# Alabuta/RaytracingInOneWeekend

Measured on AMD Instinct MI355X. Metric: Mrays/sec + frame wall-clock, huge-scene 1280x720x128spp @1/2/4/8 GPU, higher is better.
Workload: dtype f32; 1 GPU; huge-scene 1280x720x128spp (BASELINE config 3); scene=huge (486 spheres), width=1280, height=720, spp=128, max_depth=64, camera=reference, kernel=exact (bit-exact), cull, parallelism=row-interleaved x1, RCCL gather of f32 tiles, output=f32, hw_queues=8, hw_queues_env=4, deep_split=8, deep_min_items=33554432

## Files before the change

### include/rt_api.h

```cpp
#ifndef RT_API_H
#define RT_API_H

#include <stddef.h>
#include <stdint.h>

#ifdef __cplusplus
extern "C" {
#endif

#define RT_API_VERSION 2

enum rt_status {
    RT_OK = 0,
    RT_ERR_INVALID = -1,
    RT_ERR_DEVICE = -2,
    RT_ERR_CAPACITY = -3,
    RT_ERR_UNSUPPORTED = -4,
    RT_ERR_COMM = -5,
    RT_ERR_IO = -6
};

typedef struct rt_sphere {
    float center[3];
    float radius;
// ... 58 lines not shown
    uint32_t transpose_max;
    uint32_t wave_queue_rays;
    uint32_t diag;
    uint64_t ring_pass_bytes;
} rt_options;
enum rt_diag {
    RT_DIAG_IEEE_ROOTS = 1u << 0,
    RT_DIAG_NO_SHORTCUT = 1u << 1,
    RT_DIAG_NO_NEIGHBOURS = 1u << 2,
    RT_DIAG_NO_ROOT_BOX = 1u << 3,
    RT_DIAG_SHADE_LDS = 1u << 4,
    RT_DIAG_SHADE_GLOBAL = 1u << 5,
    RT_DIAG_STATS = 1u << 6,
    RT_DIAG_STATS_DEEP_ONLY = 1u << 7,
    RT_DIAG_VERBOSE = 1u << 8,
    RT_DIAG_STANDIN_TRANSPORT = 1u << 9,
    RT_DIAG_UNBOUNDED_NB = 1u << 10,
    RT_DIAG_NO_PAIRS = 1u << 11,
    RT_DIAG_PAIRS = 1u << 12,
    RT_DIAG_IN_FLIGHT = 1u << 13,
    RT_DIAG_NATURAL_ORDER = 1u << 14,
    RT_DIAG_NO_SKY = 1u << 15,
    RT_DIAG_LONE_UNSPLIT = 1u << 16,
    RT_DIAG_SKY_SERIAL = 1u << 17
};
int rt_options_default(rt_options *out);
int rt_options_parse(const char *text, rt_options *inout);
int rt_set_default_options(const rt_options *options);
int rt_get_default_options(rt_options *out);

int rt_camera_init(const float position[3], const float lookat[3], const float up[3],
                   float aspect, float vfov_degrees, float aperture, float focus_distance,
                   uint32_t mode, rt_camera *out);
int rt_camera_default(uint32_t width, uint32_t height, uint32_t mode, rt_camera *out);
int rt_scene_simple(rt_sphere *spheres, uint32_t sphere_cap, uint32_t *n_spheres,
                    rt_material *materials, uint32_t material_cap, uint32_t *n_materials);
int rt_scene_cuda(rt_sphere *spheres, uint32_t sphere_cap, uint32_t *n_spheres,
                  rt_material *materials, uint32_t material_cap, uint32_t *n_materials);
int rt_camera_cuda(uint32_t width, uint32_t height, rt_camera *out);
int rt_scene_huge(uint32_t seed, rt_sphere *spheres, uint32_t sphere_cap, uint32_t *n_spheres,
                  rt_material *materials, uint32_t material_cap, uint32_t *n_materials);

int rt_tile_order(const rt_sphere *spheres, uint32_t n_spheres, const rt_material *materials,
                  uint32_t n_materials, const rt_camera *camera, const rt_params *params,
                  uint32_t *perm, uint32_t cap, uint32_t *n_blocks, uint32_t *n_lead, uint32_t *n_sky);

int rt_release_cached(void);
int rt_render_f32(const rt_sphere *spheres, uint32_t n_spheres,
                  const rt_material *materials, uint32_t n_materials,
                  const rt_camera *camera, const rt_params *params,
                  float *rgb_out, rt_stats *stats);
int rt_render_rgb8(const rt_sphere *spheres, uint32_t n_spheres,
                   const rt_material *materials, uint32_t n_materials,
                   const rt_camera *camera, const rt_params *params,
                   uint8_t *rgb_out, rt_stats *stats);
int rt_render_multi_f32(const rt_sphere *spheres, uint32_t n_spheres,
                        const rt_material *materials, uint32_t n_materials,
                        const rt_camera *camera, const rt_params *params, int ngpu,
                        float *rgb_out, rt_stats *stats);
int rt_render_multi_rgb8(const rt_sphere *spheres, uint32_t n_spheres,
                         const rt_material *materials, uint32_t n_materials,
                         const rt_camera *camera, const rt_params *params, int ngpu,
                         uint8_t *rgb_out, rt_stats *stats);

int rt_write_ppm(const char *path, const uint8_t *rgb, uint32_t width, uint32_t height);

int rt_render_cuda_impl(uint32_t width, uint32_t height, uint8_t *rgb_out);

// ... 99 lines not shown
```

### raytracinginoneweekend_amd/__init__.py

```python
from . import _abi as abi
from ._lib import RtError, lib
from .camera import CORRECTED, REFERENCE, Camera
from .render import (DeviceScene, MultiContext, default_options, default_options_set, denoise,
                     denoise_device, denoise_params,
                     epilogue_rgb8_device, make_params, options, parse_options, render_aov, render_cuda_impl, render_f32,
                     release_cached, render_multi_f32, render_multi_rgb8, render_rgb8, save_ppm,
                     set_default_options, tile_order)
from .scene import (Dielectric, Lambert, Metal, RaytracerData, Sphere, cuda_scene_arrays, huge_scene,
                    huge_scene_arrays, simple_scene, simple_scene_arrays)

__version__ = "0.1.0"
```

### raytracinginoneweekend_amd/_abi.py

```python
import ctypes as C

import numpy as np

RT_OK = 0
RT_ERR_INVALID = -1
RT_ERR_DEVICE = -2
RT_ERR_CAPACITY = -3
RT_ERR_UNSUPPORTED = -4
RT_ERR_COMM = -5
RT_ERR_IO = -6

RT_OUTPUT_F32, RT_OUTPUT_RGB8 = 0, 1

RT_LAMBERT, RT_METAL, RT_DIELECTRIC = 0, 1, 2
RT_CAMERA_REFERENCE, RT_CAMERA_CORRECTED = 0, 1

RT_FLAG_FULL_FRAME = 1 << 0
RT_FLAG_FAST_MATH = 1 << 1
RT_FLAG_SCALAR_SCENE = 1 << 2
RT_FLAG_BRUTE_FORCE = 1 << 3
RT_FLAG_CUDA_COMPAT = 1 << 4
RT_FLAG_WAVEFRONT = 1 << 5

RT_DENOISE_DEMODULATE = 1 << 0
# ... 32 lines not shown
class RtOptions(C.Structure):
    _fields_ = [
        ("size", C.c_uint32), ("render_streams", C.c_uint32), ("workspaces_per_stream", C.c_uint32),
        ("deep_split", C.c_uint32), ("max_pass_bytes", C.c_uint64), ("max_workspace_bytes", C.c_uint64),
        ("deep_min_items", C.c_uint64), ("cluster_size", C.c_uint32), ("transpose_max", C.c_uint32),
        ("wave_queue_rays", C.c_uint32), ("diag", C.c_uint32), ("ring_pass_bytes", C.c_uint64),
    ]


class RtSceneUsage(C.Structure):
    _fields_ = [
        ("device_bytes", C.c_uint64), ("workspace_bytes", C.c_uint64), ("render_streams", C.c_uint32),
        ("workspaces", C.c_uint32), ("pass_samples", C.c_uint32), ("static_lds_bytes", C.c_uint32),
        ("max_lds_bytes", C.c_uint32), ("deep_launch", C.c_uint32), ("pair_passes", C.c_uint32),
        ("split_passes", C.c_uint32), ("lead_tiles", C.c_uint32), ("sky_tiles", C.c_uint32),
    ]


RT_DIAG = {
    "ieee_roots": 1 << 0, "no_shortcut": 1 << 1, "no_neighbours": 1 << 2, "no_root_box": 1 << 3,
    "shade_lds": 1 << 4, "shade_global": 1 << 5, "stats": 1 << 6, "stats_deep_only": 1 << 7, "verbose": 1 << 8,
    "standin_transport": 1 << 9, "unbounded_nb": 1 << 10, "no_pairs": 1 << 11, "pairs": 1 << 12,
    "in_flight": 1 << 13, "natural_order": 1 << 14, "no_sky": 1 << 15, "lone_unsplit": 1 << 16,
    "sky_serial": 1 << 17,
}


class RtStats(C.Structure):
    _fields_ = [
        ("primaries", C.c_uint64), ("segments", C.c_uint64), ("sphere_tests", C.c_uint64),
        ("box_tests", C.c_uint64),
        ("kernel_ms", C.c_double), ("wall_ms", C.c_double),
    ]


class RtAovBuffers(C.Structure):
    _fields_ = [
        ("size", C.c_uint32), ("samples", C.c_uint32),
        ("albedo", C.c_void_p), ("normal", C.c_void_p), ("depth", C.c_void_p), ("alpha", C.c_void_p),
        ("sphere_id", C.c_void_p),
    ]


class RtDenoiseParams(C.Structure):
    _fields_ = [
        ("size", C.c_uint32), ("width", C.c_uint32), ("height", C.c_uint32), ("levels", C.c_uint32),
        ("sigma_color", C.c_float), ("sigma_normal", C.c_float), ("sigma_depth", C.c_float),
# ... 59 lines not shown
```

### raytracinginoneweekend_amd/_lib.py

```python
import ctypes as C
import os

from . import _abi as abi

PKG = os.path.dirname(os.path.abspath(__file__))
LIB_PATH = os.environ.get("RT_LIB_PATH") or os.path.join(PKG, "librt_mi355x.so")

_lib = None


class RtError(RuntimeError):

    def __init__(self, status, message):
        super().__init__(f"rt status {status}: {message}")
        self.status = status


def _declare(L):
    P = C.POINTER
    sig = {
        "rt_version": (C.c_int, []),
        "rt_last_error": (C.c_char_p, []),
        "rt_device_count": (C.c_int, [P(C.c_int)]),
        "rt_camera_init": (C.c_int, [P(C.c_float), P(C.c_float), P(C.c_float), C.c_float, C.c_float,
                                     C.c_float, C.c_float, C.c_uint32, P(abi.RtCamera)]),
        "rt_camera_default": (C.c_int, [C.c_uint32, C.c_uint32, C.c_uint32, P(abi.RtCamera)]),
        "rt_scene_simple": (C.c_int, [P(abi.RtSphere), C.c_uint32, P(C.c_uint32), P(abi.RtMaterial),
                                      C.c_uint32, P(C.c_uint32)]),
        "rt_scene_huge": (C.c_int, [C.c_uint32, P(abi.RtSphere), C.c_uint32, P(C.c_uint32),
                                    P(abi.RtMaterial), C.c_uint32, P(C.c_uint32)]),
        "rt_scene_cuda": (C.c_int, [P(abi.RtSphere), C.c_uint32, P(C.c_uint32), P(abi.RtMaterial),
                                    C.c_uint32, P(C.c_uint32)]),
        "rt_camera_cuda": (C.c_int, [C.c_uint32, C.c_uint32, P(abi.RtCamera)]),
        "rt_render_cuda_impl": (C.c_int, [C.c_uint32, C.c_uint32, P(C.c_uint8)]),
        "rt_release_cached": (C.c_int, []),
        "rt_tile_order": (C.c_int, [P(abi.RtSphere), C.c_uint32, P(abi.RtMaterial), C.c_uint32, P(abi.RtCamera),
                                    P(abi.RtParams), P(C.c_uint32), C.c_uint32, P(C.c_uint32), P(C.c_uint32),
                                    P(C.c_uint32)]),
        "rt_render_f32": (C.c_int, [P(abi.RtSphere), C.c_uint32, P(abi.RtMaterial), C.c_uint32,
                                    P(abi.RtCamera), P(abi.RtParams), P(C.c_float), P(abi.RtStats)]),
        "rt_render_rgb8": (C.c_int, [P(abi.RtSphere), C.c_uint32, P(abi.RtMaterial), C.c_uint32,
                                     P(abi.RtCamera), P(abi.RtParams), P(C.c_uint8), P(abi.RtStats)]),
        "rt_render_multi_f32": (C.c_int, [P(abi.RtSphere), C.c_uint32, P(abi.RtMaterial), C.c_uint32,
                                          P(abi.RtCamera), P(abi.RtParams), C.c_int, P(C.c_float),
                                          P(abi.RtStats)]),
        "rt_render_multi_rgb8": (C.c_int, [P(abi.RtSphere), C.c_uint32, P(abi.RtMaterial), C.c_uint32,
                                           P(abi.RtCamera), P(abi.RtParams), C.c_int, P(C.c_uint8),
                                           P(abi.RtStats)]),
        "rt_write_ppm": (C.c_int, [C.c_char_p, P(C.c_uint8), C.c_uint32, C.c_uint32]),
        "rt_multi_create": (C.c_int, [P(abi.RtSphere), C.c_uint32, P(abi.RtMaterial), C.c_uint32, P(C.c_int),
                                      C.c_int, P(C.c_void_p)]),
        "rt_multi_destroy": (C.c_int, [C.c_void_p]),
        "rt_multi_info": (C.c_int, [C.c_void_p, P(C.c_int), P(C.c_int)]),
        "rt_multi_render_device": (C.c_int, [C.c_void_p, P(abi.RtCamera), P(abi.RtParams), C.c_uint32, C.c_void_p,
                                             C.c_void_p]),
        "rt_multi_render_f32": (C.c_int, [C.c_void_p, P(abi.RtCamera), P(abi.RtParams), P(C.c_float),
                                          P(abi.RtStats)]),
        "rt_multi_render_rgb8": (C.c_int, [C.c_void_p, P(abi.RtCamera), P(abi.RtParams), P(C.c_uint8),
                                           P(abi.RtStats)]),
        "rt_scene_create": (C.c_int, [P(abi.RtSphere), C.c_uint32, P(abi.RtMaterial), C.c_uint32, C.c_int,
                                      P(C.c_void_p)]),
# ... 60 lines not shown
```

### raytracinginoneweekend_amd/csrc/rt_consts.h

```cpp
#pragma once
#include <stdint.h>

namespace rt {

struct UDiv {
    uint32_t m, s1, s2;
};

constexpr float kIsoR2Grow = 1.0201f;
constexpr uint32_t kShortcut = 0x80000000u;
#ifndef RT_SUPER
#define RT_SUPER 8
#endif
constexpr uint32_t kSuperClusters = RT_SUPER;
static_assert(kSuperClusters % 2 == 0, "clusters are tested in pairs");

}
```

### raytracinginoneweekend_amd/csrc/rt_device.h

```cpp
#pragma once
#include <hip/hip_runtime.h>
#include <stdint.h>

#include "rt_consts.h"

namespace rt {

struct FrameConsts {
    float org[3], llc[3], hor[3], ver[3];
    float lens, fW, fH;
    uint32_t corrected, W, spp;
    uint32_t inc_data_lo, inc_data_hi, inc_cam_lo, inc_cam_hi;
    uint32_t row_offset, row_stride, tiled_rows, tiles_x, n_pixels, sample_begin;
    UDiv div_W, div_tiles_x, div_n_pixels;
    uint32_t tile_lw;
    float rW, rH;
    uint32_t div_fast;
    uint32_t n_pairs;
};

constexpr uint32_t kItSlot = (1u << 29) - 1u;
constexpr uint32_t kItSecond = 1u << 31;
constexpr uint32_t kItFirstDeep = 1u << 30;
constexpr uint32_t kItRestart = 1u << 29;
// ... 25 lines not shown
    uint32_t full_frame;
    uint64_t inc_data, inc_cam;
    uint32_t n_pixels, tiles_x, tiled_rows;
    uint32_t tile_lw;
    uint32_t sample_begin, sample_end;
    uint32_t n_items;
    uint32_t n_slots;
    uint32_t n_pair_items;
    uint32_t n_blocks;
    float guided_l2b;
    uint32_t n_spheres, n_materials;
    const float4 *blob;
    uint32_t blob_units;
    uint32_t n_geo, n_always, n_clusters, clus_offset;
    uint32_t n_supers, supers_offset;
    uint32_t use_root;
    uint32_t iso;
    uint32_t transpose_max;
    uint32_t fast_roots;
    float clus_pad;
    uint32_t shade_offset;
    uint32_t lds_units;
    uint32_t shade_lds;
    float *slots;
    uint32_t *queue_ctr;
    unsigned long long *segments;
    unsigned long long *dbg;
    DeepQueue deep;
    uint32_t deep_depth;
    uint32_t deep_mode;
    uint32_t deep_prio;
    uint32_t deep_static;
    uint32_t diag_unbounded_nb;
    const uint32_t *block_perm;
    uint32_t n_groups;
    uint32_t grp_pix[4];
    uint32_t grp_items[3];
    uint32_t grp_blocks[3];
    UDiv div_grp[3];
};

constexpr uint32_t kDbgError = 15;
enum BoundsCode : uint32_t {
    BC_NONE = 0, BC_HINT_NB = 1, BC_SHADE = 2, BC_SLOT = 3, BC_DEEP_APPEND = 4, BC_DEEP_ITEM = 5,
    BC_DEEP_HINT = 6, BC_MEMBERS = 7, BC_DEEP_PX = 8
};
// ... 93 lines not shown
```

### raytracinginoneweekend_amd/csrc/rt_host.cpp

```cpp
#include <dlfcn.h>
#include <hip/hip_runtime.h>
#include <rccl/rccl.h>

#include <algorithm>
#include <cerrno>
#include <cfloat>
#include <chrono>
#include <cmath>
#include <cstdint>
#include <cstdio>
#include <cstdlib>
#include <cstring>
#include <map>
#include <mutex>
#include <random>
#include <string>
#include <vector>

#include "../../include/rt_api.h"
#include "rt_device.h"
#include "rt_host_build.h"

using namespace rthost;

// ... 64 lines not shown
#define RT_SHORT_OTHERS -1
#endif
int grid_wg_per_cu(int occ, bool in_flight, uint32_t streams, uint64_t pass_items)
{
    if (!in_flight) return occ;
    const int short_others = RT_SHORT_OTHERS > 0 ? RT_SHORT_OTHERS : std::max(1, static_cast<int>(streams) - 1);
    const int others = pass_items <= kShortPassItems ? short_others
                                                     : std::min(2, std::max(1, static_cast<int>(streams) - 1));
    return std::max(1, (occ + others - 1) / others);
}

}

struct rt_scene {
    int device = 0;
    rt_options opt{};
    uint32_t n_spheres = 0, n_materials = 0;
    float *blob[2] = {nullptr, nullptr};
    uint32_t blob_units[2] = {0, 0}, n_geo[2] = {0, 0}, n_always[2] = {0, 0}, n_clusters[2] = {0, 0},
             clus_offset[2] = {0, 0};
    float clus_pad[2] = {0.f, 0.f};
    uint32_t n_supers[2] = {0, 0}, supers_offset[2] = {0, 0};
    uint32_t shade_offset[2] = {0, 0};
    bool in_fast_range = false;
    float *slots[kMaxWs] = {};
    size_t slots_bytes[kMaxWs] = {};
    float *acc = nullptr;
    size_t acc_bytes = 0;
    void *deep[kMaxWs] = {};
    size_t deep_bytes[kMaxWs] = {}, deep_clean[kMaxWs] = {};
    size_t deep_meet_at[kMaxWs] = {};
    unsigned long long *deep_over = nullptr, *deep_over_dev = nullptr;
    static constexpr size_t kDeepOffKeys = 8;
    static constexpr uint64_t kDeepOffCalls = 256;
    std::vector<std::pair<unsigned long long, uint64_t>> deep_off;
    void *wq = nullptr;
    size_t wq_bytes = 0;
    int occ_wave[2] = {-1, -1};
    uint32_t *queue_ctr = nullptr;
    hipStream_t xs[kMaxBufs] = {};
    hipEvent_t ev_done[kMaxWs] = {}, ev_free[kMaxWs] = {};
    hipEvent_t ev_main[kMaxWs] = {};
    hipEvent_t ev_sky = nullptr;
    bool free_valid[kMaxWs] = {};
    bool ctr_dirty[kMaxWs];
    rt_scene() { std::fill(std::begin(ctr_dirty), std::end(ctr_dirty), true); }
// ... 195 lines not shown

extern "C" {


int rt_scene_destroy(rt_scene *sc)
{
    if (!sc) return RT_OK;
    int prev = 0;
    (void)hipGetDevice(&prev);
    (void)hipSetDevice(sc->device);
    for (auto e : sc->ev_begin) (void)hipEventDestroy(e);
    for (auto e : sc->ev_end) (void)hipEventDestroy(e);
    for (uint32_t b = 0; b < kMaxBufs; ++b) {
        if (sc->xs[b]) (void)hipStreamSynchronize(sc->xs[b]);
        if (sc->xs[b]) (void)hipStreamDestroy(sc->xs[b]);
    }
    for (uint32_t b = 0; b < kMaxWs; ++b) {
        if (sc->ev_done[b]) (void)hipEventDestroy(sc->ev_done[b]);
        if (sc->ev_free[b]) (void)hipEventDestroy(sc->ev_free[b]);
        if (sc->ev_main[b]) (void)hipEventDestroy(sc->ev_main[b]);
    }
    if (sc->ev_tail) (void)hipEventDestroy(sc->ev_tail);
    if (sc->ev_sky) (void)hipEventDestroy(sc->ev_sky);
    for (void *p : {(void *)sc->blob[0], (void *)sc->blob[1], (void *)sc->dbg, (void *)sc->acc, (void *)sc->queue_ctr, sc->wq})
        if (p) (void)hipFree(p);
    for (float *p : sc->slots)
        if (p) (void)hipFree(p);
    for (void *p : sc->deep)
        if (p) (void)hipFree(p);
    if (sc->deep_over) (void)hipHostFree(sc->deep_over);
    for (auto &o : sc->orders)
        if (o.d_perm) (void)hipFree(o.d_perm);
    (void)hipSetDevice(prev);
    delete sc;
    return RT_OK;
}

int rt_scene_create(const rt_sphere *spheres, uint32_t n_spheres, const rt_material *materials,
                    uint32_t n_materials, int device, rt_scene **out)
{
    return rt_scene_create_ex(spheres, n_spheres, materials, n_materials, device, nullptr, out);
}

int rt_scene_create_ex(const rt_sphere *spheres, uint32_t n_spheres, const rt_material *materials,
                       uint32_t n_materials, int device, const rt_options *options, rt_scene **out)
{
    if (!out || (n_spheres && !spheres) || !materials || !n_materials)
// ... 68 lines not shown
    }
    sc->device = device;
    sc->n_spheres = n_spheres;
    sc->n_materials = n_materials;
    auto up = [&](void **dst, const void *src, size_t bytes) -> int {
        RT_HIP(hipMalloc(dst, bytes));
        RT_HIP(hipMemcpy(*dst, src, bytes, hipMemcpyHostToDevice));
        return RT_OK;
    };
    int rc = RT_OK;
    for (int b = 0; b < 2 && rc == RT_OK; ++b) {
        rc = up((void **)&sc->blob[b], blobs[b].data.data(), blobs[b].data.size() * 4);
        sc->blob_units[b] = static_cast<uint32_t>(blobs[b].data.size() / 4);
        sc->n_geo[b] = blobs[b].n_geo;
        sc->n_always[b] = blobs[b].n_always;
        sc->n_clusters[b] = blobs[b].n_clusters;
        sc->clus_offset[b] = blobs[b].clus_offset;
        sc->clus_pad[b] = blobs[b].clus_pad;
        sc->n_supers[b] = blobs[b].n_supers;
        sc->supers_offset[b] = blobs[b].supers_offset;
        sc->shade_offset[b] = blobs[b].shade_offset;
    }
    if (rc == RT_OK) {
        hipError_t e = hipMalloc((void **)&sc->queue_ctr, kCtrWords * sizeof(uint32_t));
        if (e != hipSuccess) rc = fail(RT_ERR_DEVICE, std::string("hipMalloc: ") + hipGetErrorString(e));
        if (rc == RT_OK &&
            (hipHostMalloc((void **)&sc->deep_over, kMaxWs * sizeof(unsigned long long), hipHostMallocMapped) != hipSuccess ||
             hipHostGetDevicePointer((void **)&sc->deep_over_dev, sc->deep_over, 0) != hipSuccess))
            rc = fail(RT_ERR_DEVICE, "rt_scene_create: pinned host allocation failed");
        if (rc == RT_OK) std::memset(sc->deep_over, 0, kMaxWs * sizeof(unsigned long long));
        for (uint32_t b = 0; b < kMaxWs && rc == RT_OK; ++b) {
            if ((b < kMaxBufs && hipStreamCreateWithFlags(&sc->xs[b], hipStreamNonBlocking) != hipSuccess) ||
                hipEventCreateWithFlags(&sc->ev_done[b], hipEventDisableTiming) != hipSuccess ||
                hipEventCreateWithFlags(&sc->ev_free[b], hipEventDisableTiming) != hipSuccess)
                rc = fail(RT_ERR_DEVICE, "rt_scene_create: stream/event creation failed");
        }
        if (rc == RT_OK && (hipEventCreateWithFlags(&sc->ev_tail, hipEventDisableTiming) != hipSuccess ||
                            hipEventCreateWithFlags(&sc->ev_sky, hipEventDisableTiming) != hipSuccess))
            rc = fail(RT_ERR_DEVICE, "rt_scene_create: event creation failed");
    }
    if (rc == RT_OK) {
        hipDeviceProp_t prop;
        hipError_t e = hipGetDeviceProperties(&prop, device);
        if (e != hipSuccess) rc = fail(RT_ERR_DEVICE, std::string("hipGetDeviceProperties: ") + hipGetErrorString(e));
        else {
            sc->cu_count = prop.multiProcessorCount;
// ... 184 lines not shown
        if (!sc->dbg) {
            RT_HIP(hipMalloc((void **)&sc->dbg, rt::kDbgWords * sizeof(unsigned long long)));
            RT_HIP(hipMemset(sc->dbg, 0, rt::kDbgWords * sizeof(unsigned long long)));
        }
        k.dbg = sc->dbg;
    }
    const int b = cull ? 1 : 0;
    const int cull_mode = cull ? 7 : 0;
    k.blob = reinterpret_cast<const float4 *>(sc->blob[b]);
    k.blob_units = sc->blob_units[b];
    k.n_geo = sc->n_geo[b];
    k.n_always = sc->n_always[b];
    k.n_clusters = sc->n_clusters[b];
    k.clus_offset = sc->clus_offset[b];
    k.clus_pad = sc->clus_pad[b];
    k.n_supers = sc->n_supers[b];
    k.supers_offset = sc->supers_offset[b];
    k.use_root = (O.diag & RT_DIAG_NO_ROOT_BOX) ? 0u : 1u;
    k.iso = (O.diag & RT_DIAG_NO_SHORTCUT) ? 0u : 1u;
    k.transpose_max = O.transpose_max;
    k.diag_unbounded_nb = (O.diag & RT_DIAG_UNBOUNDED_NB) ? 1u : 0u;
    k.fast_roots = sc->in_fast_range && camera_in_fast_range(*camera) && !(O.diag & RT_DIAG_IEEE_ROOTS) ? 1u : 0u;
    k.shade_offset = sc->shade_offset[b];
    auto occ_for = [&](int in_lds, int *out) -> int {
        int &o = sc->occ[variant][cull ? 1 : 0][in_lds];
        if (o < 0) {
            const size_t bytes = variant == rt::V_EXACT_SCALAR ? 0 : static_cast<size_t>(in_lds ? k.blob_units : k.shade_offset) * 16u;
            RT_HIP(rt::occupancy_render(variant, cull_mode, &o, bytes));
            o = std::max(o, 1);
        }
        *out = o;
        return RT_OK;
    };
    int occ_geo = 0, occ_all = 0;
    if (int rc = occ_for(0, &occ_geo); rc) return rc;
    if (int rc = occ_for(1, &occ_all); rc) return rc;
    const bool shade_fits = static_cast<size_t>(k.blob_units) * 16u + sc->static_lds[cull] <= sc->max_lds;
    k.shade_lds = variant != rt::V_EXACT_SCALAR && shade_fits &&
                  ((O.diag & RT_DIAG_SHADE_LDS) ? true : (O.diag & RT_DIAG_SHADE_GLOBAL) ? false : occ_all >= occ_geo);
    k.lds_units = variant == rt::V_EXACT_SCALAR ? 0u : (k.shade_lds ? k.blob_units : k.shade_offset);
    const size_t lds = static_cast<size_t>(k.lds_units) * 16u;
    const int occ = k.shade_lds ? occ_all : occ_geo;

    for (uint32_t w = 0; w < kMaxWs; ++w) {
        const unsigned long long v = __atomic_exchange_n(sc->deep_over + w, 0ull, __ATOMIC_ACQ_REL);
        if (!v) continue;
// ... 565 lines not shown
int rt_scene_kernel_times(rt_scene *sc, uint32_t max, float *ms, uint32_t *n)
{
    if (!sc || !n || (max && !ms)) return fail(RT_ERR_INVALID, "rt_scene_kernel_times: null argument");
    const uint64_t avail = std::min<uint64_t>(sc->calls, rt_scene::kRing);
    const uint32_t cnt = static_cast<uint32_t>(std::min<uint64_t>(avail, max));
    RT_HIP(hipSetDevice(sc->device));
    for (uint32_t i = 0; i < cnt; ++i) {
        const uint32_t r = static_cast<uint32_t>((sc->calls - cnt + i) % rt_scene::kRing);
        RT_HIP(hipEventSynchronize(sc->ev_end[r]));
        RT_HIP(hipEventElapsedTime(ms + i, sc->ev_begin[r], sc->ev_end[r]));
    }
    *n = cnt;
    return RT_OK;
}

int rt_scene_usage_get(const rt_scene *sc, rt_scene_usage *out)
{
    if (!sc || !out) return fail(RT_ERR_INVALID, "rt_scene_usage_get: null argument");
    rt_scene_usage u{};
    uint64_t ws = sc->acc_bytes + sc->wq_bytes;
    for (uint32_t w = 0; w < kMaxWs; ++w) ws += sc->slots_bytes[w] + sc->deep_bytes[w];
    uint64_t fixed = kCtrWords * sizeof(uint32_t) + (sc->dbg ? rt::kDbgWords * sizeof(unsigned long long) : 0u);
    for (int b = 0; b < 2; ++b) fixed += static_cast<uint64_t>(sc->blob_units[b]) * 16u;
    u.device_bytes = ws + fixed;
    u.workspace_bytes = ws;
    u.render_streams = sc->used_streams;
    u.workspaces = sc->used_ws;
    u.pass_samples = sc->used_pass;
    u.deep_launch = sc->used_deep;
    u.pair_passes = sc->used_pairs;
    u.split_passes = sc->used_split;
    u.lead_tiles = sc->used_lead;
    u.sky_tiles = sc->used_sky;
    u.static_lds_bytes = static_cast<uint32_t>(sc->static_lds[1]);
    u.max_lds_bytes = static_cast<uint32_t>(sc->max_lds);
    *out = u;
    return RT_OK;
}

int rt_scene_debug_counters(rt_scene *sc, uint64_t out[16], int reset)
{
    if (!sc || !out) return fail(RT_ERR_INVALID, "rt_scene_debug_counters: null argument");
    RT_HIP(hipSetDevice(sc->device));
    if (!sc->dbg) {
        std::memset(out, 0, 16 * sizeof(uint64_t));
        return RT_OK;
// ... 951 lines not shown
```

### raytracinginoneweekend_amd/csrc/rt_host_build.cpp

```cpp
#include "rt_host_build.h"

#include <algorithm>
#include <cerrno>
#include <cfloat>
#include <cmath>
#include <cstdint>
#include <cstdio>
#include <cstdlib>
#include <cstring>
#include <map>
#include <mutex>
#include <random>
#include <string>
#include <thread>
#include <vector>

namespace rthost {

thread_local std::string g_error;

int fail(int code, const std::string &msg)
{
    g_error = msg;
    return code;
// ... 32 lines not shown
    o.max_workspace_bytes = 0;
    o.deep_min_items = 1ull << 25;
    o.cluster_size = 16;
    o.transpose_max = 16;
    o.wave_queue_rays = 1u << 25;
    o.diag = 0;
    o.ring_pass_bytes = 384ull << 20;
    return o;
}

int check_options(const rt_options &o)
{
    auto bad = [](const char *field) { return fail(RT_ERR_INVALID, std::string("rt_options: bad ") + field); };
    if (o.size != sizeof(rt_options)) return bad("size (set it to sizeof(rt_options))");
    if (o.render_streams > kMaxBufs) return bad("render_streams (0..8)");
    if (o.workspaces_per_stream < 1 || o.workspaces_per_stream > kMaxWs / kMaxBufs) return bad("workspaces_per_stream (1..2)");
    if (o.deep_split > 1024) return bad("deep_split (0..1024)");
    if (o.max_pass_bytes < 12 || o.max_pass_bytes > kMaxSlotsBytes) return bad("max_pass_bytes (12 B..2 GiB)");
    if (o.ring_pass_bytes && (o.ring_pass_bytes < 12 || o.ring_pass_bytes > kMaxSlotsBytes))
        return bad("ring_pass_bytes (0 or 12 B..2 GiB)");
    if (o.cluster_size < 4 || o.cluster_size > 64 || o.cluster_size % 4) return bad("cluster_size (4..64, multiple of 4)");
    if (o.transpose_max > 16) return bad("transpose_max (0..16)");
    if (o.wave_queue_rays < 64) return bad("wave_queue_rays (>= 64)");
    if (o.diag & ~((RT_DIAG_SKY_SERIAL << 1) - 1u)) return bad("diag (unknown bit)");
    if ((o.diag & RT_DIAG_SHADE_LDS) && (o.diag & RT_DIAG_SHADE_GLOBAL)) return bad("diag (shade_lds with shade_global)");
    return RT_OK;
}

int parse_options(const char *text, rt_options &o)
{
    static const struct { const char *name; uint32_t bit; } kDiag[] = {
        {"ieee_roots", RT_DIAG_IEEE_ROOTS}, {"no_shortcut", RT_DIAG_NO_SHORTCUT},
        {"no_neighbours", RT_DIAG_NO_NEIGHBOURS}, {"no_root_box", RT_DIAG_NO_ROOT_BOX},
        {"shade_lds", RT_DIAG_SHADE_LDS}, {"shade_global", RT_DIAG_SHADE_GLOBAL}, {"stats", RT_DIAG_STATS},
        {"stats_deep_only", RT_DIAG_STATS_DEEP_ONLY}, {"verbose", RT_DIAG_VERBOSE},
        {"standin_transport", RT_DIAG_STANDIN_TRANSPORT}, {"unbounded_nb", RT_DIAG_UNBOUNDED_NB},
        {"no_pairs", RT_DIAG_NO_PAIRS}, {"pairs", RT_DIAG_PAIRS}, {"in_flight", RT_DIAG_IN_FLIGHT},
        {"natural_order", RT_DIAG_NATURAL_ORDER}, {"no_sky", RT_DIAG_NO_SKY}, {"lone_unsplit", RT_DIAG_LONE_UNSPLIT},
        {"sky_serial", RT_DIAG_SKY_SERIAL}};
    rt_options n = o;
    std::string all(text ? text : "");
    for (char &c : all)
        if (c == ';' || c == ' ' || c == '\t' || c == '\n') c = ',';
    size_t pos = 0;
    while (pos <= all.size()) {
        const size_t end = std::min(all.find(',', pos), all.size());
        const std::string item = all.substr(pos, end - pos);
        pos = end + 1;
        if (item.empty()) continue;
        const size_t eq = item.find('=');
        if (eq == std::string::npos || eq == 0 || eq + 1 == item.size())
            return fail(RT_ERR_INVALID, "rt_options_parse: expected key=value, got '" + item + "'");
        const std::string key = item.substr(0, eq), val = item.substr(eq + 1);
        char *stop = nullptr;
        errno = 0;
        const unsigned long long v = std::strtoull(val.c_str(), &stop, 0);
        if (errno || !stop || *stop || val[0] == '-')
            return fail(RT_ERR_INVALID, "rt_options_parse: bad value for " + key + ": '" + val + "'");
        auto u32 = [&](uint32_t &f) {
            if (v > 0xffffffffull) return false;
            f = static_cast<uint32_t>(v);
            return true;
// ... 437 lines not shown
            if (T == S) continue;
            const double rt_ = std::fabs(static_cast<double>(s[T].radius));
            double d2 = 0.0;
            for (int a = 0; a < 3; ++a) {
                const double lo = s[T].center[a] - rt_ - pad, hi = s[T].center[a] + rt_ + pad;
                const double e = C[a] < lo ? lo - C[a] : (C[a] > hi ? C[a] - hi : 0.0);
                d2 += e * e;
            }
            if (!(d2 > R * R * (1.0 + 1e-9))) {
                if (n_nb == 2 || !slots_fit || slot[T] == ~0u) {
                    ok = false;
                    break;
                }
                nb[n_nb++] = slot[T];
            }
        }
        if (ok && n_nb && nb_off) ok = false;
        if (ok)
            word[S] = rt::kShortcut | (n_nb > 0 ? nb[0] + 1u : 0u) | (n_nb > 1 ? (nb[1] + 1u) << 15 : 0u);
    }
    return word;
}

scene_geom scene_geometry(const rt_sphere *s, const blob_t &b)
{
    scene_geom g;
    for (uint32_t i : b.always) g.always.push_back(s[i]);
    g.clus_pad = b.clus_pad;
    for (uint32_t c = 0; c < b.n_clusters; ++c) {
        const float *r = b.data.data() + 4u * b.clus_offset + 8u * c;
        uint32_t packed;
        std::memcpy(&packed, r + 7, 4);
        if ((packed >> 16) == 0u || !(r[3] >= 0.f)) continue;
        g.boxes.insert(g.boxes.end(), r, r + 6);
    }
    if (b.n_clusters) {
        const float *r = b.data.data() + 4u * b.supers_offset + 8u * b.n_supers;
        if (r[3] >= 0.f) {
            std::copy(r, r + 6, g.root);
            g.has_root = true;
        }
    }
    return g;
}

namespace {
// ... 202 lines not shown
                  const rt_camera *camera, const rt_params *params, uint32_t *perm, uint32_t cap, uint32_t *n_blocks,
                  uint32_t *n_lead, uint32_t *n_sky)
{
    if ((n_spheres && !spheres) || !materials || !camera || !params || !n_blocks || !n_lead || !n_sky || (cap && !perm))
        return fail(RT_ERR_INVALID, "rt_tile_order: null argument");
    (void)n_materials;
    rt_options opt;
    if (int rc = default_options(opt); rc) return rc;
    const blob_t b = build_blob(spheres, n_spheres, true, opt.cluster_size);
    const scene_geom g = scene_geometry(spheres, b);
    const uint32_t st = params->row_stride ? params->row_stride : 1u;
    const uint32_t rows = params->num_rows ? params->num_rows
                          : params->row_offset >= params->height ? 0u
                                                                 : (params->height - params->row_offset + st - 1u) / st;
    const tile_order t = classify_tiles(*camera, params->width, params->height, params->row_offset, st, rows, 3u, g);
    *n_blocks = static_cast<uint32_t>(t.perm.size());
    *n_lead = t.n_lead;
    *n_sky = t.n_sky;
    if (t.perm.size() > cap) return cap ? fail(RT_ERR_CAPACITY, "rt_tile_order: perm buffer too small") : RT_OK;
    std::copy(t.perm.begin(), t.perm.end(), perm);
    return RT_OK;
}

int rt_write_ppm(const char *path, const uint8_t *rgb, uint32_t width, uint32_t height)
{
    if (!path || (!rgb && width && height)) return fail(RT_ERR_INVALID, "rt_write_ppm: null argument");
    std::FILE *f = std::fopen(path, "wb");
    if (!f) return fail(RT_ERR_IO, std::string("rt_write_ppm: bad file ") + path);
    const std::string hdr = "P6\n" + std::to_string(width) + " " + std::to_string(height) + "\n255\n";
    const size_t n = static_cast<size_t>(width) * height * 3u;
    const bool ok = std::fwrite(hdr.data(), 1, hdr.size(), f) == hdr.size() && (n == 0 || std::fwrite(rgb, 1, n, f) == n);
    const bool closed = std::fclose(f) == 0;
    if (!ok || !closed) return fail(RT_ERR_IO, std::string("rt_write_ppm: write failed: ") + path);
    return RT_OK;
}

}
```

### raytracinginoneweekend_amd/csrc/rt_host_build.h

```cpp
#pragma once
#include <cstdint>
#include <string>
#include <vector>

#include "../../include/rt_api.h"
#include "rt_consts.h"

namespace rthost {

extern thread_local std::string g_error;
int fail(int code, const std::string &msg);

constexpr uint64_t kMaxSlotsBytes = 1ull << 31;
static_assert(kMaxSlotsBytes / 12 < (1ull << 32), "slot index width");
constexpr uint32_t kMaxBufs = 8;
constexpr uint32_t kMaxWs = 2 * kMaxBufs + 1;

rt_options library_defaults();
int check_options(const rt_options &o);
int default_options(rt_options &out);

struct blob_t {
    std::vector<float> data;
    uint32_t n_geo = 0, n_always = 0, n_clusters = 0, clus_offset = 0, n_clusters_real = 0;
    uint32_t n_supers = 0, supers_offset = 0, shade_offset = 0;
    float clus_pad = 0.f;
    std::vector<uint32_t> always;
};
blob_t build_blob(const rt_sphere *s, uint32_t n, bool clustered, uint32_t cluster_max);
std::vector<uint32_t> shortcut_words(const rt_sphere *s, uint32_t n, const rt_material *m, const blob_t &b,
                                     bool nb_off);

struct scene_geom {
    std::vector<rt_sphere> always;
    std::vector<float> boxes;
    float root[6] = {0.f, 0.f, 0.f, -1.f, -1.f, -1.f};
    bool has_root = false;
    float clus_pad = 0.f;
};
scene_geom scene_geometry(const rt_sphere *s, const blob_t &b);
struct tile_order {
    std::vector<uint32_t> perm;
    uint32_t n_lead = 0, n_sky = 0;
};
tile_order classify_tiles(const rt_camera &cam, uint32_t W, uint32_t H, uint32_t row_offset, uint32_t row_stride,
                          uint32_t num_rows, uint32_t tile_lw, const scene_geom &g, bool sky_only = false);

rt::UDiv make_udiv(uint32_t d);
bool exact_by_reciprocal(float b);

}
```

### raytracinginoneweekend_amd/csrc/rt_kernel.hip

```cpp
#include <hip/hip_runtime.h>
#include <float.h>
#include <stdint.h>

#include "rt_device.h"

namespace rt {

#define RT_TMIN 0.008f
#define RT_TMAX FLT_MAX

struct f3 { float x, y, z; };
__device__ __forceinline__ f3 mk(float x, float y, float z) { return {x, y, z}; }
__device__ __forceinline__ f3 operator+(f3 a, f3 b) { return {a.x + b.x, a.y + b.y, a.z + b.z}; }
__device__ __forceinline__ f3 operator-(f3 a, f3 b) { return {a.x - b.x, a.y - b.y, a.z - b.z}; }
__device__ __forceinline__ f3 operator*(f3 a, f3 b) { return {a.x * b.x, a.y * b.y, a.z * b.z}; }
__device__ __forceinline__ f3 operator*(f3 a, float s) { return {a.x * s, a.y * s, a.z * s}; }
__device__ __forceinline__ f3 operator/(f3 a, float s) { return {a.x / s, a.y / s, a.z / s}; }
__device__ __forceinline__ f3 adds(f3 a, float s) { return {a.x + s, a.y + s, a.z + s}; }
__device__ __forceinline__ float dot(f3 a, f3 b) { return a.x * b.x + a.y * b.y + a.z * b.z; }
__device__ __forceinline__ float length(f3 a) { return sqrtf(a.x * a.x + a.y * a.y + a.z * a.z); }
__device__ __forceinline__ f3 normalize(f3 a)
{
    float l = length(a);
    return fabsf(l) > FLT_MIN ? a / l : a;
// ... 1146 lines not shown
                else if (nw == 2u) ++dbg.ev[EV_WALK2];
                else if (nw >= 3u && nw <= 4u) ++dbg.ev[EV_WALK4];
                else if (nw >= 5u && nw <= 8u) ++dbg.ev[EV_WALK8];
            }
            if (STATS) {
                const uint64_t nh = ballot(walk && hid == ~0u);
                if (lane == 0 && wm) ++dbg_walks;
                if (lane == 0 && nh) ++dbg_walks_nohint;
            }
            h = closest_hit<FAST, CULL, STATS, COUNT>(P, geo, sidx, clus, o, d, rd, dbg, wt, walk, wm, tw, key0);
            if (!seg) h = Hit{kNoHit};
        } else if (seg) {
            h = closest_hit<FAST, CULL, STATS, COUNT>(P, geo, sidx, clus, o, d, rd, dbg, wt, true, segm, nullptr, no_hit());
        }
        stamp(2);
        {
            const uint32_t ns = lanes(seg);
            wt.add_seg(ns);
            wt.add_sph((uint64_t)ns * P.n_always);
        }

        bool done = absorbed;
        f3 col = mk(0.f, 0.f, 0.f);
        if (alive && !defer) {
            if (!seg) {
                done = true;
            } else {
                const float t = h.t();
                uint32_t ib = h.id();
                ++depth;
                if (ib == 0xffffffffu) {
                    RT_EV(EV_SKY);
                    float uy;
                    if (rd.fd != 0u) {
                        const float l = sqrt_scaled(a);
                        const float y0 = __builtin_amdgcn_rcpf(l);
                        uy = div_ray(d.y, RayDiv{l, fmaf(fmaf(-l, y0, 1.f), y0, y0), true});
                    } else {
                        uy = normalize(d).y;
                    }
                    const float tt = .5f * uy + 1.f;
                    const f3 bg = mk(1.f, 1.f, 1.f) * (1.f - tt) + mk(.5f, .7f, 1.f) * tt;
                    col = bg * att;
                    done = true;
                } else if (depth >= P.max_depth) {
                    done = true;
// ... 32 lines not shown
                        RT_EV(EV_UNIT_DIR);
                        f3 ud;
                        if (rd.fd != 0u && all_lanes_min_abs_ok(d)) ud = div3_short(d, sqrt_scaled(a));
                        else ud = normalize(d);
                        const f3 rf = reflect(ud, hn);
                        if (kind == 1u) {
                            d = rf;
                            PN(thread_slot(wave_base)) = make_float4(hn.x, hn.y, hn.z, md.w);
                            pend = true;
                            pend_metal = true;
                        } else {
                            RT_EV(EV_DIELECTRIC);
                            const float4 dcs = dielectric_record<V>(P, blob, ib);
                            {
                                const uint32_t sl = thread_slot(wave_base);
                                PN(sl) = make_float4(sf.x, sf.y, sf.z, sf.w * sf.w);
                                const uint32_t w = __float_as_uint(dcs.w);
                                HID(sl) = ib | (w & kShortcut);
                                NB(sl) = w;
                            }
                            f3 outward = mk(-hn.x, -hn.y, -hn.z);
                            float ri = md.w, xs = dcs.y;
                            float cosv = dot(ud, hn);
                            if (cosv <= 0.f) {
                                outward = outward * -1.f;
                                ri = dcs.x;
                                xs = dcs.z;
                                cosv *= -1.f;
                            }
                            const f3 refr = refract(ud, outward, ri);
                            float prob = 1.f;
                            if (refr.x * refr.x + refr.y * refr.y + refr.z * refr.z > 0.f) prob = schlick_x(xs, cosv);
                            d = canonical(rng, inc_data) < prob ? rf : refr;
                        }
                    }
                }
            }
            stamp(3);
        }
        if (done) {
            RT_EV(EV_STORE);
            finish(col);
        }
    }

    if (COUNT && p.segments) {
        if (lane == 0) {
            atomicAdd(p.segments + 0, (unsigned long long)wt.seg);
            atomicAdd(p.segments + 1, (unsigned long long)wt.sph);
            atomicAdd(p.segments + 2, (unsigned long long)wt.box);
        }
    }
    if (STATS && p.dbg) {
        const uint32_t c[8] = {dbg_iters, dbg_refills, dbg.wave_blocks, dbg.lane_blocks, dbg.wave_roots,
                               dbg.lane_roots, lane == 0 ? (uint32_t)wt.seg : 0u, dbg.wave_member_blocks};
#pragma unroll
        for (int i = 0; i < 8; ++i) {
            unsigned long long v = c[i];
            for (int off = 32; off >= 1; off >>= 1) v += __shfl_xor(v, off);
            if (lane == 0) atomicAdd(p.dbg + i, v);
        }
// ... 708 lines not shown
```

### raytracinginoneweekend_amd/render.py

```python
import contextlib
import ctypes as C
import os

import numpy as np

from . import _abi as abi
from ._lib import check, lib
from .camera import Camera


def make_params(width, height, spp, max_depth=64, seed=1234, row_offset=0, row_stride=1, num_rows=0,
                full_frame=False, scalar_scene=False, fast_math=False, brute_force=False, cuda_compat=False,
                wavefront=False):
    flags = (abi.RT_FLAG_FULL_FRAME if full_frame else 0) | (abi.RT_FLAG_SCALAR_SCENE if scalar_scene else 0) \
        | (abi.RT_FLAG_FAST_MATH if fast_math else 0) | (abi.RT_FLAG_BRUTE_FORCE if brute_force else 0) \
        | (abi.RT_FLAG_CUDA_COMPAT if cuda_compat else 0) | (abi.RT_FLAG_WAVEFRONT if wavefront else 0)
    return abi.RtParams(width, height, spp, max_depth, seed, row_offset, row_stride, num_rows, flags)


def options(base=None, **fields):
    o = abi.RtOptions()
    if base is None:
        check(lib().rt_options_default(C.byref(o)))
    else:
# ... 136 lines not shown
    rec = denoise_buffers({**{n: a.ctypes.data for n, a in host.items()}, "out": out.ctypes.data})
    check(lib().rt_denoise(C.byref(p), C.byref(rec), C.byref(stats) if stats is not None else None))
    return out


def denoise_device(pointers, params, stream=None):
    rec = denoise_buffers(pointers)
    check(lib().rt_denoise_device(C.byref(params), C.byref(rec), C.c_void_p(stream or 0)))


def tile_order(scene, params, camera=None):
    s, m = _scene_arrays(scene)
    nb, nl, ns = C.c_uint32(0), C.c_uint32(0), C.c_uint32(0)
    args = (abi.ptr(s, C.POINTER(abi.RtSphere)), len(s), abi.ptr(m, C.POINTER(abi.RtMaterial)), len(m),
            C.byref(_cam(camera, params)), C.byref(params))
    check(lib().rt_tile_order(*args, None, 0, C.byref(nb), C.byref(nl), C.byref(ns)))
    perm = np.zeros(nb.value, dtype=np.uint32)
    if nb.value:
        check(lib().rt_tile_order(*args, abi.ptr(perm, C.POINTER(C.c_uint32)), nb.value, C.byref(nb), C.byref(nl),
                                  C.byref(ns)))
    return perm, nl.value, ns.value


def release_cached():
    check(lib().rt_release_cached())


def render_multi_f32(scene, params, ngpu=0, camera=None):
    s, m = _scene_arrays(scene)
    out = np.zeros((params.height, params.width, 3), dtype=np.float32)
    st = abi.RtStats()
    check(lib().rt_render_multi_f32(abi.ptr(s, C.POINTER(abi.RtSphere)), len(s),
                                    abi.ptr(m, C.POINTER(abi.RtMaterial)), len(m), C.byref(_cam(camera, params)),
                                    C.byref(params), ngpu, abi.ptr(out, C.POINTER(C.c_float)), C.byref(st)))
    return out, st


def render_multi_rgb8(scene, params, ngpu=0, camera=None):
    s, m = _scene_arrays(scene)
    out = np.zeros((params.height, params.width, 3), dtype=np.uint8)
    st = abi.RtStats()
    check(lib().rt_render_multi_rgb8(abi.ptr(s, C.POINTER(abi.RtSphere)), len(s),
                                     abi.ptr(m, C.POINTER(abi.RtMaterial)), len(m), C.byref(_cam(camera, params)),
                                     C.byref(params), ngpu, abi.ptr(out, C.POINTER(C.c_uint8)), C.byref(st)))
    return out, st

# ... 142 lines not shown
```

Baseline: 56940 Mrays/s.

## Terminate rays trapped by total internal reflection inside isolated dielectric spheres

```diff
diff --git a/include/rt_api.h b/include/rt_api.h
--- a/include/rt_api.h
+++ b/include/rt_api.h
@@ -104,7 +104,8 @@
     RT_DIAG_NATURAL_ORDER = 1u << 14,
     RT_DIAG_NO_SKY = 1u << 15,
     RT_DIAG_LONE_UNSPLIT = 1u << 16,
-    RT_DIAG_SKY_SERIAL = 1u << 17
+    RT_DIAG_SKY_SERIAL = 1u << 17,
+    RT_DIAG_NO_TRAP_END = 1u << 19
 };
 int rt_options_default(rt_options *out);
 int rt_options_parse(const char *text, rt_options *inout);
@@ -126,6 +127,9 @@
 int rt_tile_order(const rt_sphere *spheres, uint32_t n_spheres, const rt_material *materials,
                   uint32_t n_materials, const rt_camera *camera, const rt_params *params,
                   uint32_t *perm, uint32_t cap, uint32_t *n_blocks, uint32_t *n_lead, uint32_t *n_sky);
+
+int rt_trap_windows(const rt_sphere *spheres, uint32_t n_spheres, const rt_material *materials,
+                    uint32_t n_materials, float *out);
 
 int rt_release_cached(void);
 int rt_render_f32(const rt_sphere *spheres, uint32_t n_spheres,
diff --git a/raytracinginoneweekend_amd/__init__.py b/raytracinginoneweekend_amd/__init__.py
--- a/raytracinginoneweekend_amd/__init__.py
+++ b/raytracinginoneweekend_amd/__init__.py
@@ -5,7 +5,7 @@
                      denoise_device, denoise_params,
                      epilogue_rgb8_device, make_params, options, parse_options, render_aov, render_cuda_impl, render_f32,
                      release_cached, render_multi_f32, render_multi_rgb8, render_rgb8, save_ppm,
-                     set_default_options, tile_order)
+                     set_default_options, tile_order, trap_windows)
 from .scene import (Dielectric, Lambert, Metal, RaytracerData, Sphere, cuda_scene_arrays, huge_scene,
                     huge_scene_arrays, simple_scene, simple_scene_arrays)
 
diff --git a/raytracinginoneweekend_amd/_abi.py b/raytracinginoneweekend_amd/_abi.py
--- a/raytracinginoneweekend_amd/_abi.py
+++ b/raytracinginoneweekend_amd/_abi.py
@@ -78,7 +78,7 @@
     "shade_lds": 1 << 4, "shade_global": 1 << 5, "stats": 1 << 6, "stats_deep_only": 1 << 7, "verbose": 1 << 8,
     "standin_transport": 1 << 9, "unbounded_nb": 1 << 10, "no_pairs": 1 << 11, "pairs": 1 << 12,
     "in_flight": 1 << 13, "natural_order": 1 << 14, "no_sky": 1 << 15, "lone_unsplit": 1 << 16,
-    "sky_serial": 1 << 17,
+    "sky_serial": 1 << 17, "no_trap_end": 1 << 19,
 }
 
 
diff --git a/raytracinginoneweekend_amd/_lib.py b/raytracinginoneweekend_amd/_lib.py
--- a/raytracinginoneweekend_amd/_lib.py
+++ b/raytracinginoneweekend_amd/_lib.py
@@ -37,6 +37,7 @@
         "rt_tile_order": (C.c_int, [P(abi.RtSphere), C.c_uint32, P(abi.RtMaterial), C.c_uint32, P(abi.RtCamera),
                                     P(abi.RtParams), P(C.c_uint32), C.c_uint32, P(C.c_uint32), P(C.c_uint32),
                                     P(C.c_uint32)]),
+        "rt_trap_windows": (C.c_int, [P(abi.RtSphere), C.c_uint32, P(abi.RtMaterial), C.c_uint32, P(C.c_float)]),
         "rt_render_f32": (C.c_int, [P(abi.RtSphere), C.c_uint32, P(abi.RtMaterial), C.c_uint32,
                                     P(abi.RtCamera), P(abi.RtParams), P(C.c_float), P(abi.RtStats)]),
         "rt_render_rgb8": (C.c_int, [P(abi.RtSphere), C.c_uint32, P(abi.RtMaterial), C.c_uint32,
diff --git a/raytracinginoneweekend_amd/csrc/rt_consts.h b/raytracinginoneweekend_amd/csrc/rt_consts.h
--- a/raytracinginoneweekend_amd/csrc/rt_consts.h
+++ b/raytracinginoneweekend_amd/csrc/rt_consts.h
@@ -9,6 +9,8 @@
 
 constexpr float kIsoR2Grow = 1.0201f;
 constexpr uint32_t kShortcut = 0x80000000u;
+constexpr uint32_t kTrapDepth = 64;
+constexpr double kTrapDriftK = 1.0;
 #ifndef RT_SUPER
 #define RT_SUPER 8
 #endif
diff --git a/raytracinginoneweekend_amd/csrc/rt_device.h b/raytracinginoneweekend_amd/csrc/rt_device.h
--- a/raytracinginoneweekend_amd/csrc/rt_device.h
+++ b/raytracinginoneweekend_amd/csrc/rt_device.h
@@ -71,6 +71,7 @@
     uint32_t shade_offset;
     uint32_t lds_units;
     uint32_t shade_lds;
+    const float2 *trap;
     float *slots;
     uint32_t *queue_ctr;
     unsigned long long *segments;
diff --git a/raytracinginoneweekend_amd/csrc/rt_host.cpp b/raytracinginoneweekend_amd/csrc/rt_host.cpp
--- a/raytracinginoneweekend_amd/csrc/rt_host.cpp
+++ b/raytracinginoneweekend_amd/csrc/rt_host.cpp
@@ -110,6 +110,7 @@
     float clus_pad[2] = {0.f, 0.f};
     uint32_t n_supers[2] = {0, 0}, supers_offset[2] = {0, 0};
     uint32_t shade_offset[2] = {0, 0};
+    float *trap = nullptr;
     bool in_fast_range = false;
     float *slots[kMaxWs] = {};
     size_t slots_bytes[kMaxWs] = {};
@@ -351,7 +352,7 @@
     }
     if (sc->ev_tail) (void)hipEventDestroy(sc->ev_tail);
     if (sc->ev_sky) (void)hipEventDestroy(sc->ev_sky);
-    for (void *p : {(void *)sc->blob[0], (void *)sc->blob[1], (void *)sc->dbg, (void *)sc->acc, (void *)sc->queue_ctr, sc->wq})
+    for (void *p : {(void *)sc->blob[0], (void *)sc->blob[1], (void *)sc->dbg, (void *)sc->acc, (void *)sc->queue_ctr, sc->wq, (void *)sc->trap})
         if (p) (void)hipFree(p);
     for (float *p : sc->slots)
         if (p) (void)hipFree(p);
@@ -466,6 +467,17 @@
         sc->shade_offset[b] = blobs[b].shade_offset;
     }
     if (rc == RT_OK) {
+        std::vector<float> trap = trap_windows(spheres, n_spheres, materials);
+        const size_t nw = std::max<size_t>(n_spheres, 1u);
+        trap.resize(4 * nw);
+        for (size_t i = (opt.diag & RT_DIAG_NO_TRAP_END) ? 0 : nw; i < 2 * nw; ++i) {
+            trap[2 * i] = 1.f;
+            trap[2 * i + 1] = 0.f;
+        }
+        if (n_spheres == 0) { trap[0] = 1.f; trap[1] = 0.f; }
+        rc = up((void **)&sc->trap, trap.data(), trap.size() * sizeof(float));
+    }
+    if (rc == RT_OK) {
         hipError_t e = hipMalloc((void **)&sc->queue_ctr, kCtrWords * sizeof(uint32_t));
         if (e != hipSuccess) rc = fail(RT_ERR_DEVICE, std::string("hipMalloc: ") + hipGetErrorString(e));
         if (rc == RT_OK &&
@@ -696,6 +708,8 @@
     k.diag_unbounded_nb = (O.diag & RT_DIAG_UNBOUNDED_NB) ? 1u : 0u;
     k.fast_roots = sc->in_fast_range && camera_in_fast_range(*camera) && !(O.diag & RT_DIAG_IEEE_ROOTS) ? 1u : 0u;
     k.shade_offset = sc->shade_offset[b];
+    k.trap = reinterpret_cast<const float2 *>(sc->trap) +
+             (P.max_depth > rt::kTrapDepth ? std::max<size_t>(sc->n_spheres, 1u) : 0u);
     auto occ_for = [&](int in_lds, int *out) -> int {
         int &o = sc->occ[variant][cull ? 1 : 0][in_lds];
         if (o < 0) {
@@ -1307,6 +1321,7 @@
     for (uint32_t w = 0; w < kMaxWs; ++w) ws += sc->slots_bytes[w] + sc->deep_bytes[w];
     uint64_t fixed = kCtrWords * sizeof(uint32_t) + (sc->dbg ? rt::kDbgWords * sizeof(unsigned long long) : 0u);
     for (int b = 0; b < 2; ++b) fixed += static_cast<uint64_t>(sc->blob_units[b]) * 16u;
+    fixed += static_cast<uint64_t>(std::max(sc->n_spheres, 1u)) * 16u;
     u.device_bytes = ws + fixed;
     u.workspace_bytes = ws;
     u.render_streams = sc->used_streams;
diff --git a/raytracinginoneweekend_amd/csrc/rt_host_build.cpp b/raytracinginoneweekend_amd/csrc/rt_host_build.cpp
--- a/raytracinginoneweekend_amd/csrc/rt_host_build.cpp
+++ b/raytracinginoneweekend_amd/csrc/rt_host_build.cpp
@@ -78,7 +78,7 @@
     if (o.cluster_size < 4 || o.cluster_size > 64 || o.cluster_size % 4) return bad("cluster_size (4..64, multiple of 4)");
     if (o.transpose_max > 16) return bad("transpose_max (0..16)");
     if (o.wave_queue_rays < 64) return bad("wave_queue_rays (>= 64)");
-    if (o.diag & ~((RT_DIAG_SKY_SERIAL << 1) - 1u)) return bad("diag (unknown bit)");
+    if (o.diag & ~(((RT_DIAG_SKY_SERIAL << 1) - 1u) | RT_DIAG_NO_TRAP_END)) return bad("diag (unknown bit)");
     if ((o.diag & RT_DIAG_SHADE_LDS) && (o.diag & RT_DIAG_SHADE_GLOBAL)) return bad("diag (shade_lds with shade_global)");
     return RT_OK;
 }
@@ -93,7 +93,7 @@
         {"standin_transport", RT_DIAG_STANDIN_TRANSPORT}, {"unbounded_nb", RT_DIAG_UNBOUNDED_NB},
         {"no_pairs", RT_DIAG_NO_PAIRS}, {"pairs", RT_DIAG_PAIRS}, {"in_flight", RT_DIAG_IN_FLIGHT},
         {"natural_order", RT_DIAG_NATURAL_ORDER}, {"no_sky", RT_DIAG_NO_SKY}, {"lone_unsplit", RT_DIAG_LONE_UNSPLIT},
-        {"sky_serial", RT_DIAG_SKY_SERIAL}};
+        {"sky_serial", RT_DIAG_SKY_SERIAL}, {"no_trap_end", RT_DIAG_NO_TRAP_END}};
     rt_options n = o;
     std::string all(text ? text : "");
     for (char &c : all)
@@ -577,6 +577,49 @@
     return word;
 }
 
+std::vector<float> trap_windows(const rt_sphere *s, uint32_t n, const rt_material *m)
+{
+    std::vector<float> win(2 * static_cast<size_t>(n));
+    for (uint32_t i = 0; i < n; ++i) {
+        win[2 * i] = 1.f;
+        win[2 * i + 1] = 0.f;
+    }
+    size_t n_diel = 0;
+    for (uint32_t i = 0; i < n; ++i)
+        if (m[s[i].material].kind == RT_DIELECTRIC) ++n_diel;
+    if (static_cast<double>(n_diel) * static_cast<double>(n) > 4e8) return win;
+    for (uint32_t S = 0; S < n; ++S) {
+        const rt_material &mt = m[s[S].material];
+        if (mt.kind != RT_DIELECTRIC) continue;
+        const double ior = mt.param, r = s[S].radius;
+        const double C[3] = {s[S].center[0], s[S].center[1], s[S].center[2]};
+        if (!(ior > 1.0) || !std::isfinite(ior) || !(r > 0.0) || !std::isfinite(r)) continue;
+        if (!std::isfinite(C[0]) || !std::isfinite(C[1]) || !std::isfinite(C[2])) continue;
+        const double R = r * std::sqrt(static_cast<double>(rt::kIsoR2Grow));
+        bool isolated = true;
+        for (uint32_t T = 0; T < n && isolated; ++T) {
+            if (T == S) continue;
+            const double rT = std::fabs(static_cast<double>(s[T].radius));
+            const double dx = s[T].center[0] - C[0], dy = s[T].center[1] - C[1], dz = s[T].center[2] - C[2];
+            const double dist = std::sqrt(dx * dx + dy * dy + dz * dz);
+            if (!(std::fabs(dist - rT) > R * (1.0 + 1e-9))) isolated = false;
+        }
+        if (!isolated) continue;
+        const double cinf = std::max(std::fabs(C[0]), std::max(std::fabs(C[1]), std::fabs(C[2])));
+        const double margin = rt::kTrapDriftK * rt::kTrapDepth * 0x1p-23 * (cinf + r) / static_cast<double>(0.008f);
+        const double lo = static_cast<double>(0.008f) * (1.0 + 1e-3) / (2.0 * r) + margin;
+        const double hi = std::sqrt(1.0 - 1.0 / (ior * ior)) - margin;
+        if (!(lo <= hi) || !(lo > 0.0) || !(hi < 1.0)) continue;
+        float flo = static_cast<float>(lo), fhi = static_cast<float>(hi);
+        if (static_cast<double>(flo) < lo) flo = std::nextafter(flo, 2.f);
+        if (static_cast<double>(fhi) > hi) fhi = std::nextafter(fhi, -1.f);
+        if (!(flo <= fhi)) continue;
+        win[2 * S] = flo;
+        win[2 * S + 1] = fhi;
+    }
+    return win;
+}
+
 scene_geom scene_geometry(const rt_sphere *s, const blob_t &b)
 {
     scene_geom g;
@@ -825,6 +868,18 @@
     return RT_OK;
 }
 
+int rt_trap_windows(const rt_sphere *spheres, uint32_t n_spheres, const rt_material *materials, uint32_t n_materials,
+                    float *out)
+{
+    if ((n_spheres && (!spheres || !out)) || !materials || !n_materials)
+        return fail(RT_ERR_INVALID, "rt_trap_windows: null argument or no materials");
+    for (uint32_t i = 0; i < n_spheres; ++i)
+        if (spheres[i].material >= n_materials) return fail(RT_ERR_INVALID, "rt_trap_windows: bad material index");
+    const std::vector<float> w = trap_windows(spheres, n_spheres, materials);
+    std::copy(w.begin(), w.end(), out);
+    return RT_OK;
+}
+
 int rt_write_ppm(const char *path, const uint8_t *rgb, uint32_t width, uint32_t height)
 {
     if (!path || (!rgb && width && height)) return fail(RT_ERR_INVALID, "rt_write_ppm: null argument");
diff --git a/raytracinginoneweekend_amd/csrc/rt_host_build.h b/raytracinginoneweekend_amd/csrc/rt_host_build.h
--- a/raytracinginoneweekend_amd/csrc/rt_host_build.h
+++ b/raytracinginoneweekend_amd/csrc/rt_host_build.h
@@ -30,6 +30,7 @@
 blob_t build_blob(const rt_sphere *s, uint32_t n, bool clustered, uint32_t cluster_max);
 std::vector<uint32_t> shortcut_words(const rt_sphere *s, uint32_t n, const rt_material *m, const blob_t &b,
                                      bool nb_off);
+std::vector<float> trap_windows(const rt_sphere *s, uint32_t n, const rt_material *m);
 
 struct scene_geom {
     std::vector<rt_sphere> always;
diff --git a/raytracinginoneweekend_amd/csrc/rt_kernel.hip b/raytracinginoneweekend_amd/csrc/rt_kernel.hip
--- a/raytracinginoneweekend_amd/csrc/rt_kernel.hip
+++ b/raytracinginoneweekend_amd/csrc/rt_kernel.hip
@@ -1192,6 +1192,7 @@
 
         bool done = absorbed;
         f3 col = mk(0.f, 0.f, 0.f);
+        uint32_t trap_rem = 0;
         if (alive && !defer) {
             if (!seg) {
                 done = true;
@@ -1270,6 +1271,7 @@
                             f3 outward = mk(-hn.x, -hn.y, -hn.z);
                             float ri = md.w, xs = dcs.y;
                             float cosv = dot(ud, hn);
+                            const bool inside = cosv > 0.f;
                             if (cosv <= 0.f) {
                                 outward = outward * -1.f;
                                 ri = dcs.x;
@@ -1278,13 +1280,28 @@
                             }
                             const f3 refr = refract(ud, outward, ri);
                             float prob = 1.f;
-                            if (refr.x * refr.x + refr.y * refr.y + refr.z * refr.z > 0.f) prob = schlick_x(xs, cosv);
+                            const float rn = refr.x * refr.x + refr.y * refr.y + refr.z * refr.z;
+                            if (rn > 0.f) {
+                                prob = schlick_x(xs, cosv);
+                            } else if (inside && rn != rn) {
+                                const __attribute__((address_space(1))) float *win =
+                                    (const __attribute__((address_space(1))) float *)(P.trap + ib);
+                                if (cosv >= win[0] && cosv <= win[1]) {
+                                    done = true;
+                                    if (COUNT) trap_rem = P.max_depth - depth;
+                                }
+                            }
                             d = canonical(rng, inc_data) < prob ? rf : refr;
                         }
                     }
                 }
             }
             stamp(3);
+        }
+        if constexpr (COUNT) {
+            uint32_t r = trap_rem;
+            for (int off = 32; off >= 1; off >>= 1) r += (uint32_t)__shfl_xor((int)r, off);
+            wt.add_seg(r);
         }
         if (done) {
             RT_EV(EV_STORE);
diff --git a/raytracinginoneweekend_amd/render.py b/raytracinginoneweekend_amd/render.py
--- a/raytracinginoneweekend_amd/render.py
+++ b/raytracinginoneweekend_amd/render.py
@@ -182,6 +182,14 @@
     return perm, nl.value, ns.value
 
 
+def trap_windows(scene):
+    s, m = _scene_arrays(scene)
+    out = np.zeros((len(s), 2), dtype=np.float32)
+    check(lib().rt_trap_windows(abi.ptr(s, C.POINTER(abi.RtSphere)), len(s), abi.ptr(m, C.POINTER(abi.RtMaterial)),
+                                len(m), abi.ptr(out, C.POINTER(C.c_float))))
+    return out
+
+
 def release_cached():
     check(lib().rt_release_cached())
 
```

Measured after the change: 60280 Mrays/s (median of 6 runs). 5.9% higher.
